# ruppelb/Large-Scale-ViT-SLAM

Hardware: AMD Instinct MI355X
Metric: chunks/sec (16-frame 518x518) + ViT MFMA util% (higher is better)
Workload: dtype bf16; 1 GPU; VGGT aggregator forward (DINOv2-L/14-reg + 24x frame/global AA blocks), 1 chunk of 16 frames 518x518, layers 4/11/17/23 emitted; frames=16, parallelism=replicas x1

## Files before the change

### include/vggt_mi355x.h

```cpp
#ifndef VGGT_MI355X_H
#define VGGT_MI355X_H

#include <stddef.h>
#include <stdint.h>

#ifdef __cplusplus
extern "C" {
#endif

#define VGGT_OK 0
#define VGGT_ERR_SHAPE (-1)
#define VGGT_ERR_ALIGN (-2)
#define VGGT_ERR_HIP (-3)
#define VGGT_ERR_UNSUPPORTED (-4)

#define VGGT_DTYPE_F32 0
#define VGGT_DTYPE_BF16 1

#define VGGT_EPI_BF16 0
#define VGGT_EPI_GELU_BF16 1
#define VGGT_EPI_RESID_F32 2
#define VGGT_EPI_F32 3

#define VGGT_ROPE_NONE 0
#define VGGT_ROPE_2D 1
#define VGGT_ROPE_1D 2

const char* vggt_version(void);

#define VGGT_TUNE_GEMM_TILE 1
#define VGGT_TUNE_ATTN_WAVES 2
#define VGGT_TUNE_ATTN_VARIANT 3
#define VGGT_TUNE_CONV_PF2 4
#define VGGT_TUNE_ATTN16 5
#define VGGT_TUNE_LINEAR_ONE_LAUNCH 6
#define VGGT_TUNE_LINEAR_SPLIT_K 7
#define VGGT_TUNE_LINEAR_WK 8
#define VGGT_TUNE_GEMM_BALANCE 10
#define VGGT_TUNE_ATTN_TAIL_SPLIT 11
int vggt_tune(int knob, int value);

#define VGGT_STREAM_SHORT_WORKGROUPS 1
int vggt_set_stream_config(void* stream, int cus, int flags);

int vggt_gemm_bf16(const void* A, int64_t lda, const void* W, int64_t ldw, const float* bias, int M, int N, int K,
                   int epi, void* out, int64_t ldo, const float* gamma, float* out2, int64_t ldo2, void* stream);

int vggt_gemm_bf16_gelu_pre(const void* A, int64_t lda, const void* W, int64_t ldw, const float* bias, int M, int N,
                            int K, void* out, int64_t ldo, void* pre, int64_t ldp, void* stream);

int vggt_gemm_qkv(const void* A, int64_t lda, const void* W, int64_t ldw, const float* bias, int M, int H, int D, int K,
                  void* out, int64_t ldo, const float* qw, const float* qb, const float* kw, const float* kb, float eps,
                  int rope_mode, const int32_t* pos, int period, const float* cos_tab, const float* sin_tab,
                  int tab_len, void* stream);

int vggt_gemm_headnorm(const void* A, int64_t lda, const void* W, int64_t ldw, const float* bias, int M, int N, int H,
                       int D, int K, void* out, int64_t ldo, const float* nw, const float* nb, float eps, int rope_mode,
                       const int32_t* pos, int period, const float* cos_tab, const float* sin_tab, int tab_len,
                       void* stream);

int vggt_layernorm(const void* x, int in_dtype, int64_t ldx, const float* w, const float* b, float eps, int M, int C,
                   void* y, int out_dtype, int64_t ldy, void* stream);

int vggt_resid_add_layernorm(float* x, int64_t ldx, const void* y, int64_t ldy, const float* gamma, float* out2,
                             int64_t ldo2, const float* w, const float* b, float eps, int M, int C, void* xn,
                             int64_t ldn, void* stream);

int vggt_resid_add_layernorm_nostore(const float* x, int64_t ldx, const void* y, int64_t ldy, const float* gamma,
                                     const float* w, const float* b, float eps, int M, int C, void* xn, int64_t ldn,
                                     void* stream);
int vggt_resid_add2_layernorm(float* x, int64_t ldx, const void* y, int64_t ldy, const float* gamma, const void* y2,
                              int64_t ldy2, const float* gamma2, float* out2, int64_t ldo2, const float* w,
                              const float* b, float eps, int M, int C, void* xn, int64_t ldn, void* stream);

int vggt_headnorm_rope(void* buf, int64_t ld, int col_off, int M, int H, int D, const float* w, const float* b,
                       float eps, int rope_mode, const int32_t* pos, int period, const float* cos_tab,
                       const float* sin_tab, int tab_len, void* stream);

int vggt_qknorm_rope(void* qkv, int64_t ld, int M, int H, int D, const float* qw, const float* qb, const float* kw,
                     const float* kb, float eps, int rope_mode, const int32_t* pos, int period, const float* cos_tab,
                     const float* sin_tab, int tab_len, void* stream);

int vggt_qknorm_rope_out(const void* src, int64_t lds, void* dst, int64_t ldd, int M, int H, int D, const float* qw,
                         const float* qb, const float* kw, const float* kb, float eps, int rope_mode,
                         const int32_t* pos, int period, const float* cos_tab, const float* sin_tab, int tab_len,
                         void* stream);
int vggt_headnorm_rope_out(const void* src, int64_t lds, void* dst, int64_t ldd, int M, int H, int D, const float* w,
                           const float* b, float eps, int rope_mode, const int32_t* pos, int period,
                           const float* cos_tab, const float* sin_tab, int tab_len, void* stream);

int vggt_attention_fwd(const void* q, int64_t ldq, int64_t q_bstride, const void* k, int64_t ldk, int64_t k_bstride,
                       const void* v, int64_t ldv, int64_t v_bstride, void* o, int64_t ldo, int64_t o_bstride,
                       int batch, int heads, int nq, int nk, int D, float scale, void* stream);

int vggt_attention_fwd_ws(const void* q, int64_t ldq, int64_t q_bstride, const void* k, int64_t ldk,
                          int64_t k_bstride, const void* v, int64_t ldv, int64_t v_bstride, void* o, int64_t ldo,
                          int64_t o_bstride, int batch, int heads, int nq, int nk, int D, float scale, void* ws,
                          size_t ws_bytes, void* stream);
size_t vggt_attention_ws_bytes(int batch, int heads, int nq, int nk, int D, void* stream);
int vggt_attention_split_plan(int batch, int heads, int nq, int nk, int D, int cus, int* tail_blocks, int* parts);

int vggt_patch_im2col(const float* images, int F, int H, int W, int patch, const float* mean, const float* std_,
                      void* A, int Kp, void* stream);

int vggt_dino_assemble(const void* patch, const float* cls, const float* reg, const float* pos, int F, int hw,
                       int nreg, int C, float* x, void* stream);

int vggt_special_tokens(float* x, int64_t ldx, int F, int S, int P, int n, int C, const float* tok, void* stream);

int vggt_copy_rows_f32(const float* src, int64_t lds, float* dst, int64_t ldd, int rows, int cols, void* stream);

int vggt_layernorm_grouped(const void* x, int in_dtype, int64_t ldx, const float* w, const float* b, float eps, int M,
                           int C, void* y, int out_dtype, int64_t ldy, int group, int x_group_stride,
                           int x_row_offset, int y_group_stride, int y_row_offset, void* stream);

int vggt_linear_f32(const float* A, int64_t lda, const float* W, int64_t ldw, const float* bias, int M, int N, int K,
                    int act_in, int epi, float* out, int64_t ldo, const float* gamma, void* stream);
int vggt_linear_f32_grouped(const float* A, int64_t lda, int64_t a_gstride, const float* W, int64_t ldw,
                            int64_t w_gstride, const float* bias, int64_t b_gstride, int M, int N, int K, int groups,
                            int act_in, int epi, float* out, int64_t ldo, int64_t o_gstride, void* stream);
int vggt_gated_update_prep(const float* memory, const float* update, int B, int Nt, int D, float* inp, float* g_in,
                           void* stream);
// ... 150 lines not shown
```

### large-scale-vit-slam_amd/aligned_vggt/_native.py

```python
from __future__ import annotations

import ctypes
import os
from typing import Optional

import torch

from .runtime import Workspace, scratch_table

_PKG_ROOT = os.path.dirname(os.path.dirname(os.path.abspath(__file__)))
LIB_PATH = os.environ.get("VGGT_MI355X_LIB", os.path.join(_PKG_ROOT, "lib", "libvggt_mi355x.so"))
HEADER_PATH = os.path.join(os.path.dirname(_PKG_ROOT), "include", "vggt_mi355x.h")

VGGT_OK, VGGT_ERR_SHAPE, VGGT_ERR_ALIGN, VGGT_ERR_HIP, VGGT_ERR_UNSUPPORTED = 0, -1, -2, -3, -4
DTYPE_F32, DTYPE_BF16 = 0, 1
EPI_BF16, EPI_GELU_BF16, EPI_RESID_F32, EPI_F32 = 0, 1, 2, 3
ROPE_NONE, ROPE_2D, ROPE_1D = 0, 1, 2

_ERR = {VGGT_ERR_SHAPE: "unsupported or inconsistent shape", VGGT_ERR_ALIGN: "misaligned pointer or leading dimension",
        VGGT_ERR_HIP: "HIP launch/runtime error", VGGT_ERR_UNSUPPORTED: "unsupported mode or dtype"}

_vp, _i, _i64, _f = ctypes.c_void_p, ctypes.c_int, ctypes.c_int64, ctypes.c_float
_SIGS = {
    "vggt_tune": [_i, _i],
# ... 45 lines not shown
    "vggt_upsample_bilinear_split_sep": [_vp, _i, _i, _i, _i, _vp, _i, _i, _vp, _vp, _vp, _i, _vp],
    "vggt_conv2d_upsample_bf16x3": [_vp, _i, _i, _i, _i, _vp, _i, _i, _vp, _vp, _vp, _i, _i, _vp, _i64, _vp, _vp,
                                    _i64, _i, _vp],
    "vggt_split_act_bf16x2": [_vp, _i64, _i64, _i, _i, _vp, _vp, _vp],
    "vggt_upsample_bilinear_f32": [_vp, _i, _i, _i, _i, _vp, _i, _i, _vp, _vp],
    "vggt_dpt_activate": [_vp, _i64, _i64, _i, _i, _i, _vp, _vp, _vp, _vp],
    "vggt_irls_sim3": [_vp, _i64, _vp, _i64, _vp, _i64, _vp, _i64, _i, _i64, _f, _f, _i, _f, _vp, _vp, _vp, _vp,
                       ctypes.c_size_t, _vp],
    "vggt_sim3_points": [_vp, _i64, _i, _i64, _vp, _vp, _vp, _i64, _vp],
    "vggt_scale_f32": [_vp, _i64, _i, _i64, _vp, _vp],
    "vggt_pose_compose": [_vp, _vp, _vp, _vp, _i, _vp, _i, _i, _i, _i, _i, _vp, _vp, _vp],
    "vggt_attention_fwd_lse": [_vp, _i64, _i64, _vp, _i64, _i64, _vp, _i64, _i64, _vp, _i64, _i64, _vp, _i, _i, _i,
                               _i, _i, _f, _vp],
    "vggt_attention_bwd": [_vp, _i64, _i64, _vp, _i64, _i64, _vp, _i64, _vp, _vp, _i64, _i64, _vp, _vp, _vp, _i64,
                           _vp, _vp, _i64, _i, _i, _i, _i, _i, _f, _vp],
    "vggt_attention_small_bwd": [_vp, _i64, _i64, _vp, _i64, _i64, _vp, _i64, _vp, _i64, _i64, _vp, _i64, _i64, _vp,
                                 _vp, _i64, _i64, _i, _i, _i, _i, _i, _i, _f, _vp],
    "vggt_layernorm_bwd": [_vp, _i, _i64, _vp, _f, _vp, _i, _i64, _vp, _i, _i64, _i, _i, _i, _i, _i, _i, _i, _i, _vp,
                           _vp, _vp, ctypes.c_size_t, _vp],
    "vggt_headnorm_rope_bwd": [_vp, _i64, _vp, _i64, _i, _i, _i, _i, _i, _vp, _vp, _f, _i, _vp, _i, _vp, _vp, _i, _vp,
                               _vp, _vp, _vp, _vp, ctypes.c_size_t, _vp],
    "vggt_colsum": [_vp, _i, _i64, _i, _i, _vp, _i, _vp, ctypes.c_size_t, _vp],
    "vggt_layerscale_bwd": [_vp, _i64, _vp, _i, _i64, _vp, _vp, _i, _i64, _i, _i, _vp, _vp, _vp, ctypes.c_size_t,
                            _vp],
    "vggt_gelu_fwd": [_vp, _i, _i64, _vp, _i, _i64, _i, _i, _vp],
    "vggt_gelu_bwd": [_vp, _i, _i64, _vp, _i, _i64, _vp, _i, _i64, _i, _i, _vp, _vp, ctypes.c_size_t, _vp],
    "vggt_resid_scale_add": [_vp, _i64, _vp, _i, _i64, _vp, _i, _i, _vp],
    "vggt_gemm_bf16_gelu_pre": [_vp, _i64, _vp, _i64, _vp, _i, _i, _i, _vp, _i64, _vp, _i64, _vp],
    "vggt_resid_scale_add_from": [_vp, _i64, _vp, _i64, _vp, _i, _i64, _vp, _i, _i, _vp],
    "vggt_qknorm_rope_out": [_vp, _i64, _vp, _i64, _i, _i, _i, _vp, _vp, _vp, _vp, _f, _i, _vp, _i, _vp, _vp, _i, _vp],
    "vggt_headnorm_rope_out": [_vp, _i64, _vp, _i64, _i, _i, _i, _vp, _vp, _f, _i, _vp, _i, _vp, _vp, _i, _vp],
    "vggt_transpose_b16": [_vp, _i64, _i, _i, _vp, _i64, _i, _vp],
    "vggt_wgrad_f32": [_vp, _i64, _vp, _i64, _i, _i, _i, _vp, _i64, _i, _vp],
    "vggt_wgrad_bias_f32": [_vp, _i64, _vp, _i64, _i, _i, _i, _vp, _i64, _vp, _i, _vp],
    "vggt_wgrad_bf16": [_vp, _i64, _vp, _i64, _i, _i, _i, _vp, _i64, _i, _vp, ctypes.c_size_t, _vp],
    "vggt_batch_dot_f32": [_vp, _vp, _i64, _i, _i64, _vp, _vp, ctypes.c_size_t, _vp],
}
_WS_FNS = {"vggt_colred_workspace_bytes": [_i, _i], "vggt_layernorm_bwd_workspace_bytes": [_i, _i],
           "vggt_headnorm_rope_bwd_workspace_bytes": [_i, _i], "vggt_batch_dot_workspace_bytes": [_i, _i64],
           "vggt_wgrad_bf16_workspace_bytes": [_i, _i, _i], "vggt_attention_ws_bytes": [_i, _i, _i, _i, _i, _vp]}

_lib = None

EVENT_HOOK = None


def lib() -> ctypes.CDLL:
    global _lib
    if _lib is None:
        if not os.path.exists(LIB_PATH):
            raise RuntimeError(f"libvggt_mi355x.so not found at {LIB_PATH}: build it with "
                               f"`make -C large-scale-vit-slam_amd/csrc` (or __graft_entry__.build()); "
                               f"there is no CPU fallback for the HIP hot path")
        L = ctypes.CDLL(LIB_PATH)
        for name, argt in _SIGS.items():
            fn = getattr(L, name)
            fn.argtypes = argt
            fn.restype = ctypes.c_int
        L.vggt_version.restype = ctypes.c_char_p
        L.vggt_irls_workspace_bytes.argtypes = [_i]
        L.vggt_irls_workspace_bytes.restype = ctypes.c_size_t
        for name, argt in _WS_FNS.items():
            fn = getattr(L, name)
            fn.argtypes = argt
            fn.restype = ctypes.c_size_t
        _lib = L
    return _lib


def version() -> str:
    return lib().vggt_version().decode()


TUNE_GEMM_TILE = 1
TUNE_ATTN_WAVES = 2
TUNE_ATTN_VARIANT = 3
TUNE_CONV_PF2 = 4
TUNE_ATTN16 = 5
TUNE_LINEAR_ONE_LAUNCH = 6
TUNE_LINEAR_SPLIT_K = 7
TUNE_LINEAR_WK = 8
TUNE_GEMM_BALANCE = 10
TUNE_ATTN_TAIL_SPLIT = 11


def tune(knob: int, value: int) -> int:
    rc = lib().vggt_tune(knob, value)
    if rc == VGGT_ERR_UNSUPPORTED:
        raise ValueError(f"vggt_tune: unsupported knob/value ({knob}, {value})")
    return rc


STREAM_SHORT_WORKGROUPS = 1


def set_stream_config(stream: int, cus: int, flags: int = 0) -> int:
    rc = lib().vggt_set_stream_config(ctypes.c_void_p(stream), cus, flags)
    if rc < 0:
        raise ValueError(f"vggt_set_stream_config: rejected ({rc})")
    return rc


def mfma_probe(iters: int = 200_000, random: bool = True, seconds: float = 2.0, device=None) -> dict:
    import statistics
    device = torch.device(device or "cuda")
    ncu = torch.cuda.get_device_properties(device).multi_processor_count
    g = torch.Generator(device="cpu").manual_seed(0)
    n = ncu * 256 * 16
    ops = (torch.randn(n, generator=g) if random else torch.zeros(n)).to(torch.bfloat16).to(device)
    stamps = torch.zeros(ncu * 4, dtype=torch.int64, device=device)
    sink = torch.empty(ncu * 256, dtype=torch.float32, device=device)
    st = ctypes.c_void_p(torch.cuda.current_stream(device).cuda_stream)
    launch = lambda: _check(lib().vggt_mfma_probe(_p(stamps), _p(sink), _p(ops), ncu, iters, st),
                            "vggt_mfma_probe")
    import time
    t_end = time.perf_counter() + seconds
    while time.perf_counter() < t_end:
        launch()
        torch.cuda.synchronize(device)
    a = torch.cuda.Event(enable_timing=True)
    b = torch.cuda.Event(enable_timing=True)
    a.record()
    launch()
    b.record()
    b.synchronize()
    ms = a.elapsed_time(b)
    sp = stamps.view(ncu, 4).cpu().tolist()
    clocks = [(t1 - t0) / (r1 - r0) * 100e6 for t0, t1, r0, r1 in sp if r1 > r0]
    clk = statistics.median(clocks)
    flop = ncu * 4 * iters * 8 * 32768.0
    return {"tflops": round(flop / (ms * 1e-3) / 1e12, 1), "clock_ghz": round(clk / 1e9, 3),
            "flop_per_cycle_per_cu": round(flop / ncu / (ms * 1e-3 * clk), 1), "ms": round(ms, 3), "cus": ncu,
            "operands": "random bf16" if random else "zeros"}


def _check(rc: int, name: str) -> None:
    if rc != VGGT_OK:
        raise RuntimeError(f"{name}: {_ERR.get(rc, 'error')} (code {rc})")


def _dev(t: torch.Tensor, name: str) -> None:
    if t.device.type != "cuda":
        raise RuntimeError(f"{name}: tensor on {t.device}; the MI355X hot path runs on HIP devices only")


def _p(t: Optional[torch.Tensor]):
    return None if t is None else ctypes.c_void_p(t.data_ptr())


def _stream() -> ctypes.c_void_p:
    return ctypes.c_void_p(torch.cuda.current_stream().cuda_stream)


def _ld(t: torch.Tensor) -> int:
    if t.dim() != 2 or t.stride(1) != 1:
        raise RuntimeError("expected a 2-D row-major (unit inner stride) view")
    return t.stride(0)


def gemm_bf16(a: torch.Tensor, w: torch.Tensor, bias: torch.Tensor, out: torch.Tensor, epi: int,
              gamma: Optional[torch.Tensor] = None, out2: Optional[torch.Tensor] = None) -> torch.Tensor:
    _dev(a, "gemm_bf16")
    M, K = a.shape
    N = w.shape[0]
    assert a.dtype == torch.bfloat16 and w.dtype == torch.bfloat16 and w.shape[1] == K
    assert out.shape[0] == M and out.shape[1] == N
# ... 705 lines not shown
```

### large-scale-vit-slam_amd/csrc/attention.hip

```cpp
#include <math.h>
#include <stdlib.h>
#include <string.h>

#include <algorithm>
#include <mutex>
#include <type_traits>
#include <vector>

#include "common.h"
#include "tune.h"

namespace {

typedef __attribute__((ext_vector_type(4))) short s16x4;
typedef __attribute__((ext_vector_type(8))) short s16x8;
typedef int int32x4 __attribute__((ext_vector_type(4)));

constexpr int BKV = 64;
constexpr float THR = 8.0f;

struct AttnArgs {
  const bf16_t* q;
  const bf16_t* k;
  const bf16_t* v;
// ... 554 lines not shown
        }
      }
      return nt;
    };
    if constexpr (VAR & 32) {
      const int t1 = run(std::true_type{}, 0);
      if (t1 < nt) run(std::false_type{}, t1);
    } else {
      run(std::false_type{}, 0);
    }
  }

  if constexpr (VAR & 8) {
    l_run = lsum[0];
  } else {
    const auto sw = __builtin_amdgcn_permlane32_swap(__float_as_uint(l_run), __float_as_uint(l_run), false, false);
    l_run = __uint_as_float(sw[0]) + __uint_as_float(sw[1]);
  }
  if constexpr (SPLIT) {
    if (slab >= 0) {
      float* sp = a.ws + (int64_t)slab * SPLIT_SLAB;
#pragma unroll
      for (int db = 0; db < NDB; ++db)
#pragma unroll
        for (int gq = 0; gq < 4; ++gq)
          *(f32x4*)(sp + ((wave * (NDB * 4) + db * 4 + gq) * 64 + lane) * 4) =
              f32x4{o[db][4 * gq], o[db][4 * gq + 1], o[db][4 * gq + 2], o[db][4 * gq + 3]};
      if (hl == 0) *(f32x2*)(sp + BQ * D + (wave * 32 + lane) * 2) = f32x2{m_run, l_run};
      return;
    }
  }
  float inv = 1.f / l_run;
  if constexpr ((VAR & 32) && (VAR & 64)) {
    const auto sw = __builtin_amdgcn_permlane32_swap(__float_as_uint(lb_run), __float_as_uint(lb_run), false, false);
    inv = 1.f / (__uint_as_float(sw[0]) + __uint_as_float(sw[1]));
  }
  if constexpr (VAR & 1024) {
    VGGT_SEG(-1);
    st_acc[6] = st_prev;
    if (lane == 0) {
      unsigned long long* out = (unsigned long long*)(void*)a.lse + ((int64_t)blockIdx.x * NW + wave) * STAMP_N;
#pragma unroll
      for (int i = 0; i < STAMP_N; ++i) out[i] = st_acc[i];
    }
  } else {
    if (a.lse && hl == 0 && qrow < a.nq) a.lse[((int64_t)b * a.heads + h) * a.nq + qrow] = m_run + __log2f(l_run);
  }
  if (qrow < a.nq) {
    bf16_t* op = a.o + ((int64_t)b * a.obs + qrow) * a.ldo + h * D;
#pragma unroll
    for (int db = 0; db < NDB; ++db)
#pragma unroll
      for (int gq = 0; gq < 4; ++gq) {
        uint2 pk;
        pk.x = pack_bf2(o[db][4 * gq] * inv, o[db][4 * gq + 1] * inv);
        pk.y = pack_bf2(o[db][4 * gq + 2] * inv, o[db][4 * gq + 3] * inv);
        *(uint2*)(op + db * 32 + 8 * gq + 4 * hl) = pk;
      }
  }
}

__device__ __forceinline__ int k16_swz(int row, int chunk) { return chunk ^ ((row >> 1) & 7); }
__device__ __forceinline__ int v16_swz(int row, int chunk) { return chunk ^ (((row >> 1) & 3) << 1); }

template <int NW>
__global__ __launch_bounds__(NW * 64, 16 / NW) void attn16_fwd_kernel(AttnArgs a) {
  constexpr int D = 64;
  constexpr int BQ = NW * 32;
  constexpr int ROWB = D * 2;
  constexpr int TILEB = BKV * ROWB;
  constexpr int RPI = 1024 / ROWB;
  constexpr int CPR = ROWB / 16;
  constexpr int IPW = TILEB / 1024 / NW;
  __shared__ __attribute__((aligned(16))) char smem[2 * 2 * TILEB];
  __shared__ int redo;

  const int lane = threadIdx.x & 63;
  const int wave = __builtin_amdgcn_readfirstlane(threadIdx.x >> 6);
  const int g = lane >> 4, c16 = lane & 15;
  if constexpr (NW == 8) {
    if (wave >= 4) __builtin_amdgcn_s_setprio(1);
  }
  const int nqb = (a.nq + BQ - 1) / BQ;
  const int bid = xcd_remap(blockIdx.x, nqb * a.heads * a.batch);
  const int qblk = bid % nqb;
  const int bh = bid / nqb;
  const int h = bh % a.heads;
  const int b = bh / a.heads;

  const bf16_t* qp = a.q + (int64_t)b * a.qbs * a.ldq + h * D;
  const bf16_t* kp = a.k + (int64_t)b * a.kbs * a.ldk + h * D;
  const bf16_t* vp = a.v + (int64_t)b * a.vbs * a.ldv + h * D;
  const int q0 = qblk * BQ + wave * 32 + c16;

  bf16x8 qf[2][2];
#pragma unroll
  for (int qb = 0; qb < 2; ++qb) {
    const int qr = min(q0 + 16 * qb, a.nq - 1);
#pragma unroll
    for (int ks = 0; ks < 2; ++ks) {
      qf[qb][ks] = *(const bf16x8*)(qp + (int64_t)qr * a.ldq + ks * 32 + 8 * g);
#pragma unroll
      for (int j = 0; j < 8; ++j) qf[qb][ks][j] = (__bf16)((float)qf[qb][ks][j] * a.c);
    }
  }
#pragma unroll
  for (int qb = 0; qb < 2; ++qb)
#pragma unroll
    for (int ks = 0; ks < 2; ++ks) asm volatile("" : "+v"(qf[qb][ks]));

  uint32_t koff[IPW], voff[IPW];
#pragma unroll
  for (int i = 0; i < IPW; ++i) {
    const int row = (wave * IPW + i) * RPI + lane / CPR;
    const int cp = lane % CPR;
    koff[i] = (uint32_t)(row * a.ldk + k16_swz(row, cp) * 8) * 2u;
    voff[i] = (uint32_t)(row * a.ldv + v16_swz(row, cp) * 8) * 2u;
  }
  const uint32_t lds0 = __builtin_amdgcn_readfirstlane((uint32_t)(uintptr_t)LDS_PTR(smem)) + wave * IPW * 1024;
  const int kstep = BKV * (int)a.ldk * 2, vstep = BKV * (int)a.ldv * 2;
  const int kbytes = a.nk * (int)a.ldk * 2, vbytes = a.nk * (int)a.ldv * 2;
  auto stage = [&](int buf, int t) {
    const int ko = kstep * t, vo = vstep * t;
    const int32x4 kr = make_rsrc((const char*)kp + ko, (uint32_t)max(kbytes - ko, 0));
    const int32x4 vr = make_rsrc((const char*)vp + vo, (uint32_t)max(vbytes - vo, 0));
    const uint32_t d = lds0 + buf * 2 * TILEB;
#pragma unroll
    for (int i = 0; i < IPW; ++i) {
      dma16(kr, koff[i], d + i * 1024);
      dma16(vr, voff[i], d + TILEB + i * 1024);
    }
  };

  uint32_t ka[2];
#pragma unroll
  for (int ks = 0; ks < 2; ++ks) ka[ks] = c16 * ROWB + (k16_swz(c16, 4 * ks + g) << 4);
  uint32_t va[4];
  {
    const int qq = (lane >> 2) & 3, pp = lane & 3;
    const int r0 = 4 * g + qq;
#pragma unroll
    for (int db = 0; db < 4; ++db) {
      const int col = db * 16 + 4 * pp;
      va[db] = TILEB + r0 * ROWB + (v16_swz(r0, col >> 3) << 4) + (col & 7) * 2;
    }
  }
  const int nt = (a.nk + BKV - 1) / BKV;

  struct S8 {
    f32x4 v[4][2];
  };
  auto scores = [&](auto bufc, int t) -> S8 {
    constexpr int BUF = decltype(bufc)::value;
    const char* base = smem + BUF * 2 * TILEB;
    S8 s;
#pragma unroll
    for (int kb = 0; kb < 4; ++kb) {
      const bf16x8 k0 = *(const bf16x8*)(base + ka[0] + kb * 16 * ROWB);
      const bf16x8 k1 = *(const bf16x8*)(base + ka[1] + kb * 16 * ROWB);
#pragma unroll
      for (int qb = 0; qb < 2; ++qb) {
        s.v[kb][qb] = __builtin_amdgcn_mfma_f32_16x16x32_bf16(k0, qf[qb][0], f32x4{}, 0, 0, 0);
        s.v[kb][qb] = __builtin_amdgcn_mfma_f32_16x16x32_bf16(k1, qf[qb][1], s.v[kb][qb], 0, 0, 0);
      }
    }
    const int kv0 = t * BKV;
    if (kv0 + BKV > a.nk) {
#pragma unroll
      for (int kb = 0; kb < 4; ++kb)
#pragma unroll
        for (int i = 0; i < 4; ++i)
          if (kv0 + kb * 16 + 4 * g + i >= a.nk) {
            s.v[kb][0][i] = -INFINITY;
            s.v[kb][1][i] = -INFINITY;
          }
    }
    return s;
  };

  f32x4 o[4][2];
  float l[2];
  float m[2] = {0.f, 0.f};

  auto soft_pv = [&](auto bufc, int t, auto shc) {
    constexpr int BUF = decltype(bufc)::value;
    constexpr bool SHIFT = decltype(shc)::value;
    const char* base = smem + BUF * 2 * TILEB;
    const S8 s = scores(bufc, t);
    bf16x8 pf[2][2];
#pragma unroll
    for (int qb = 0; qb < 2; ++qb) {
      float rs = 0.f;
#pragma unroll
      for (int kk = 0; kk < 2; ++kk) {
        bf16x8 tv;
#pragma unroll
        for (int j = 0; j < 8; ++j) {
          float x = s.v[2 * kk + (j >> 2)][qb][j & 3];
          if constexpr (SHIFT) x -= m[qb];
          const float p = __builtin_amdgcn_exp2f(x);
          rs += p;
          tv[j] = (__bf16)p;
        }
        pf[qb][kk] = tv;
      }
      l[qb] += rs;
    }
    const char* vb = base;
#pragma unroll
    for (int kk = 0; kk < 2; ++kk)
#pragma unroll
      for (int db = 0; db < 4; ++db) {
        const char* p0 = vb + va[db] + kk * 32 * ROWB;
        const s16x4 lo = __builtin_amdgcn_ds_read_tr16_b64_v4i16((__attribute__((address_space(3))) s16x4*)LDS_PTR(p0));
        const s16x4 hi =
            __builtin_amdgcn_ds_read_tr16_b64_v4i16((__attribute__((address_space(3))) s16x4*)LDS_PTR(p0 + 16 * ROWB));
        const bf16x8 vf = __builtin_bit_cast(bf16x8, (s16x8)__builtin_shufflevector(lo, hi, 0, 1, 2, 3, 4, 5, 6, 7));
#pragma unroll
        for (int qb = 0; qb < 2; ++qb)
          o[db][qb] = __builtin_amdgcn_mfma_f32_16x16x32_bf16(vf, pf[qb][kk], o[db][qb], 0, 0, 0);
      }
  };

  using I0 = std::integral_constant<int, 0>;
  using I1 = std::integral_constant<int, 1>;
  auto sweep = [&](auto body) {
    stage(0, 0);
    asm volatile("s_waitcnt vmcnt(0)" ::: "memory");
    __syncthreads();
    for (int t = 0; t < nt; t += 2) {
      if (t + 1 < nt) stage(1, t + 1);
      body(I0{}, t);
      asm volatile("s_waitcnt vmcnt(0)" ::: "memory");
      __syncthreads();
      if (t + 1 >= nt) break;
      if (t + 2 < nt) stage(0, t + 2);
      body(I1{}, t + 1);
      asm volatile("s_waitcnt vmcnt(0)" ::: "memory");
      __syncthreads();
    }
  };
  auto reset = [&]() {
#pragma unroll
    for (int db = 0; db < 4; ++db)
#pragma unroll
      for (int qb = 0; qb < 2; ++qb) o[db][qb] = f32x4{};
    l[0] = l[1] = 0.f;
  };
  auto allsum = [](float x) {
    const auto s16 = __builtin_amdgcn_permlane16_swap(__float_as_uint(x), __float_as_uint(x), false, false);
    x = __uint_as_float(s16[0]) + __uint_as_float(s16[1]);
    const auto s32 = __builtin_amdgcn_permlane32_swap(__float_as_uint(x), __float_as_uint(x), false, false);
    return __uint_as_float(s32[0]) + __uint_as_float(s32[1]);
  };
  auto allmax = [](float x) {
    const auto s16 = __builtin_amdgcn_permlane16_swap(__float_as_uint(x), __float_as_uint(x), false, false);
    x = fmaxf(__uint_as_float(s16[0]), __uint_as_float(s16[1]));
    const auto s32 = __builtin_amdgcn_permlane32_swap(__float_as_uint(x), __float_as_uint(x), false, false);
    return fmaxf(__uint_as_float(s32[0]), __uint_as_float(s32[1]));
  };

  if (threadIdx.x == 0) redo = 0;
  reset();
  sweep([&](auto bufc, int t) { soft_pv(bufc, t, std::false_type{}); });
  l[0] = allsum(l[0]);
  l[1] = allsum(l[1]);
  const bool bad = !(l[0] >= 0x1p-60f && l[0] <= 0x1p100f) || !(l[1] >= 0x1p-60f && l[1] <= 0x1p100f);
  if (__builtin_amdgcn_ballot_w64(bad) != 0 && lane == 0) redo = 1;
  __syncthreads();
  if (redo) {
    float mx[2] = {-INFINITY, -INFINITY};
    sweep([&](auto bufc, int t) {
      const S8 s = scores(bufc, t);
#pragma unroll
      for (int qb = 0; qb < 2; ++qb)
#pragma unroll
        for (int kb = 0; kb < 4; ++kb)
          mx[qb] = fmaxf(fmaxf(mx[qb], fmaxf(s.v[kb][qb][0], s.v[kb][qb][1])), fmaxf(s.v[kb][qb][2], s.v[kb][qb][3]));
    });
    m[0] = allmax(mx[0]);
    m[1] = allmax(mx[1]);
    reset();
    sweep([&](auto bufc, int t) { soft_pv(bufc, t, std::true_type{}); });
    l[0] = allsum(l[0]);
    l[1] = allsum(l[1]);
  }

#pragma unroll
  for (int qb = 0; qb < 2; ++qb) {
    const int qrow = q0 + 16 * qb;
    const float inv = 1.f / l[qb];
    if (a.lse && g == 0 && qrow < a.nq) a.lse[((int64_t)b * a.heads + h) * a.nq + qrow] = m[qb] + __log2f(l[qb]);
    if (qrow < a.nq) {
      bf16_t* op = a.o + ((int64_t)b * a.obs + qrow) * a.ldo + h * D;
#pragma unroll
      for (int db = 0; db < 4; ++db) {
        uint2 pk;
        pk.x = pack_bf2(o[db][qb][0] * inv, o[db][qb][1] * inv);
        pk.y = pack_bf2(o[db][qb][2] * inv, o[db][qb][3] * inv);
        *(uint2*)(op + db * 16 + 4 * g) = pk;
      }
    }
  }
}

__global__ __launch_bounds__(256) void attn_split_merge_kernel(AttnArgs a, int n_tail) {
  constexpr int D = 64;
  const int tid = blockIdx.x * 256 + threadIdx.x;
  const int lane = tid & 63, c = (tid >> 6) & 7, wave = (tid >> 9) & 7, tu = tid >> 12;
  if (tu >= n_tail) return;
  const int nqb = (a.nq + SPLIT_BQ - 1) / SPLIT_BQ;
  const int bid = a.n_full + tu;
  const int qb = bid % nqb, bh = bid / nqb;
  const int h = bh % a.heads, b = bh / a.heads;
  const int r = wave * 32 + (lane & 31), hl = lane >> 5;
  const int qrow = qb * SPLIT_BQ + r;
  if (qrow >= a.nq) return;
  const float* sp = a.ws + (int64_t)tu * a.parts * SPLIT_SLAB;
  float mx = -INFINITY;
  for (int p = 0; p < a.parts; ++p) mx = fmaxf(mx, sp[(int64_t)p * SPLIT_SLAB + SPLIT_BQ * D + r * 2]);
  f32x4 num = f32x4{0.f, 0.f, 0.f, 0.f};
  float den = 0.f;
  for (int p = 0; p < a.parts; ++p) {
    const float* pp = sp + (int64_t)p * SPLIT_SLAB;
    const f32x2 ml = *(const f32x2*)(pp + SPLIT_BQ * D + r * 2);
    const float w = __builtin_amdgcn_exp2f(ml[0] - mx);
    num += w * *(const f32x4*)(pp + ((wave * 8 + c) * 64 + lane) * 4);
    den += w * ml[1];
  }
  const float inv = 1.f / den;
  uint2 pk;
  pk.x = pack_bf2(num[0] * inv, num[1] * inv);
  pk.y = pack_bf2(num[2] * inv, num[3] * inv);
  bf16_t* op = a.o + ((int64_t)b * a.obs + qrow) * a.ldo + h * D;
  *(uint2*)(op + (c >> 2) * 32 + 8 * (c & 3) + 4 * hl) = pk;
}

inline int attn_cu_count(hipStream_t s) {
  static int dev_cus = [] {
    int dev = 0, n = 0;
    if (hipGetDevice(&dev) != hipSuccess ||
        hipDeviceGetAttribute(&n, hipDeviceAttributeMultiprocessorCount, dev) != hipSuccess || n <= 0)
      n = 256;
    return n;
  }();
  const int n = vggt_stream_cu_count(s);
  return n > 0 ? n : dev_cus;
}

constexpr double PLAN_UNIT_OVH = 2.0;
constexpr double PLAN_TILE_US = 1.87, PLAN_BYTES_PER_US = 3.5e6, PLAN_MERGE_US = 5.0;
constexpr double PLAN_MIN_GAIN = 0.03;
constexpr int PLAN_MIN_PART_TILES = 86;

struct PlanSeg {
  int count;
  double len;
};
double plan_makespan(int cus, const PlanSeg* segs, int nseg) {
  std::vector<double> rem((size_t)cus * 2, 0.0);
  std::vector<int> cnt((size_t)cus, 0);
  int seg = 0, left = nseg > 0 ? segs[0].count : 0, resident = 0;
  double now = 0.0;
  auto more = [&]() {
    while (seg < nseg && left == 0) {
      ++seg;
      if (seg < nseg) left = segs[seg].count;
    }
    return seg < nseg;
  };
  for (;;) {
    for (int want = 0; want < 2; ++want)
      for (int cu = 0; cu < cus; ++cu)
        if (cnt[cu] == want && more()) {
          rem[cu * 2 + cnt[cu]] = segs[seg].len;
          ++cnt[cu];
          --left;
          ++resident;
        }
    if (resident == 0) return now;
    double dt = 1e300;
    for (int cu = 0; cu < cus; ++cu)
      for (int i = 0; i < cnt[cu]; ++i) dt = std::min(dt, rem[cu * 2 + i] * cnt[cu] * 0.5);
    now += dt;
    for (int cu = 0; cu < cus; ++cu) {
      const int n = cnt[cu];
      const double done = dt * 2.0 / (n > 0 ? n : 1);
      int keep = 0;
      for (int i = 0; i < n; ++i) {
        const double r = rem[cu * 2 + i] - done;
        if (r > 1e-9) rem[cu * 2 + keep++] = r;
        else --resident;
      }
      cnt[cu] = keep;
    }
  }
}

inline void split_shape(int nt, int want, int* parts, int* part_tiles) {
  const int p = std::max(1, std::min(want, nt));
  *part_tiles = (nt + p - 1) / p;
  *parts = (nt + *part_tiles - 1) / *part_tiles;
}

}

extern "C" int vggt_attention_split_plan(int batch, int heads, int nq, int nk, int D, int cus, int* tail_blocks,
                                         int* parts) {
  if (tail_blocks) *tail_blocks = 0;
  if (parts) *parts = 0;
  if (batch <= 0 || heads <= 0 || nq < 4096 || nk <= 0 || D != 64 || cus <= 0) return 0;
  const int64_t units64 = (int64_t)((nq + SPLIT_BQ - 1) / SPLIT_BQ) * heads * batch;
  const int slots = 2 * cus, nt = (nk + BKV - 1) / BKV;
  if (units64 < slots || units64 > (1 << 24) || units64 % slots == 0 || nt < 2) return 0;
  const int units = (int)units64, tail = units % slots;
  struct Entry {
    int key[4], tail, parts;
  };
  static std::mutex mu;
  static std::vector<Entry> cache;
  const int key[4] = {units, nq, nk, cus};
  std::lock_guard<std::mutex> lk(mu);
  const Entry* hit = nullptr;
  for (const Entry& e : cache)
    if (!memcmp(e.key, key, sizeof key)) hit = &e;
  if (!hit) {
    const PlanSeg whole[1] = {{units, nt + PLAN_UNIT_OVH}};
    const double t0 = plan_makespan(cus, whole, 1);
    double best = t0;
    int best_p = 0;
    for (int want = 2; want <= 4; ++want) {
      int p, pt;
// ... 13 lines not shown
  if (hit->parts < 2) return 0;
  if (tail_blocks) *tail_blocks = hit->tail;
  if (parts) *parts = hit->parts;
  return 1;
}

namespace {
void tail_split_of(int batch, int heads, int nq, int nk, int cus, int* tail, int* parts, int* part_tiles) {
  *tail = *parts = *part_tiles = 0;
  const int knob = g_vggt_attn_tail_split;
  const int64_t units = (int64_t)((nq + SPLIT_BQ - 1) / SPLIT_BQ) * heads * batch;
  const int nt = (nk + BKV - 1) / BKV;
  int t = 0, p = 0;
  if (knob < 0 || units > (1 << 18)) return;
  if (knob > 0) {
    p = knob & 0xff;
    t = (int)std::min<int64_t>(knob >> 8, units);
  } else if (!vggt_attention_split_plan(batch, heads, nq, nk, 64, cus, &t, &p)) {
    return;
  }
  int pr, pt;
  split_shape(nt, std::min(p, 4), &pr, &pt);
  if (pr < 2 || t <= 0) return;
  *tail = t;
  *parts = pr;
  *part_tiles = pt;
}

bool attn_split_path(int nq, int D) {
  static const bool dma_half = getenv("VGGT_ATTN_DMA_HALF") ? atoi(getenv("VGGT_ATTN_DMA_HALF")) != 0 : true;
  return dma_half && g_vggt_attn_variant == 33 && D == 64 && g_vggt_attn_waves == 8 && nq >= 4096;
}
}

extern "C" size_t vggt_attention_ws_bytes(int batch, int heads, int nq, int nk, int D, void* stream) {
  if (batch <= 0 || heads <= 0 || nq <= 0 || nk <= 0 || !attn_split_path(nq, D)) return 0;
  int tail, parts, pt;
  tail_split_of(batch, heads, nq, nk, attn_cu_count((hipStream_t)stream), &tail, &parts, &pt);
  return (size_t)tail * parts * SPLIT_SLAB * sizeof(float);
}

static int attention_fwd_impl(const void* q, int64_t ldq, int64_t q_bstride, const void* k, int64_t ldk,
                              int64_t k_bstride, const void* v, int64_t ldv, int64_t v_bstride, void* o, int64_t ldo,
                              int64_t o_bstride, int batch, int heads, int nq, int nk, int D, float scale, void* ws,
                              size_t ws_bytes, void* stream);

extern "C" int vggt_attention_fwd(const void* q, int64_t ldq, int64_t q_bstride, const void* k, int64_t ldk,
                                  int64_t k_bstride, const void* v, int64_t ldv, int64_t v_bstride, void* o,
                                  int64_t ldo, int64_t o_bstride, int batch, int heads, int nq, int nk, int D,
                                  float scale, void* stream) {
  return attention_fwd_impl(q, ldq, q_bstride, k, ldk, k_bstride, v, ldv, v_bstride, o, ldo, o_bstride, batch, heads,
                            nq, nk, D, scale, nullptr, 0, stream);
}

extern "C" int vggt_attention_fwd_ws(const void* q, int64_t ldq, int64_t q_bstride, const void* k, int64_t ldk,
                                     int64_t k_bstride, const void* v, int64_t ldv, int64_t v_bstride, void* o,
                                     int64_t ldo, int64_t o_bstride, int batch, int heads, int nq, int nk, int D,
                                     float scale, void* ws, size_t ws_bytes, void* stream) {
  if (ws && (uintptr_t)ws % 16) return VGGT_ERR_ALIGN;
  return attention_fwd_impl(q, ldq, q_bstride, k, ldk, k_bstride, v, ldv, v_bstride, o, ldo, o_bstride, batch, heads,
                            nq, nk, D, scale, ws, ws_bytes, stream);
}

static int attention_fwd_impl(const void* q, int64_t ldq, int64_t q_bstride, const void* k, int64_t ldk,
                              int64_t k_bstride, const void* v, int64_t ldv, int64_t v_bstride, void* o, int64_t ldo,
                              int64_t o_bstride, int batch, int heads, int nq, int nk, int D, float scale, void* ws,
                              size_t ws_bytes, void* stream) {
  if (batch <= 0 || heads <= 0 || nq <= 0 || nk <= 0) return VGGT_ERR_SHAPE;
  if (D != 64 && D != 128) return VGGT_ERR_UNSUPPORTED;
  if ((ldq | ldk | ldv | ldo) % 8 || ((uintptr_t)q | (uintptr_t)k | (uintptr_t)v | (uintptr_t)o) % 16)
    return VGGT_ERR_ALIGN;
  if ((uint64_t)nk * (uint64_t)(ldk > ldv ? ldk : ldv) * 2 >= (1ull << 31)) return VGGT_ERR_SHAPE;
  AttnArgs a{(const bf16_t*)q, (const bf16_t*)k, (const bf16_t*)v, (bf16_t*)o, ldq, ldk, ldv, ldo,
             q_bstride, k_bstride, v_bstride, o_bstride, batch, heads, nq, nk,
             scale * 1.4426950408889634f, nullptr};
  const bool two_ok = (g_vggt_attn_variant & 32) && (g_vggt_attn_variant & 65) == 1;
  const int nw = (g_vggt_attn_waves == 8 && nq >= 4096) ? 8 : (g_vggt_attn_waves == 2 && two_ok) ? 2 : 4;
  const int nwg = ((nq + nw * 32 - 1) / (nw * 32)) * heads * batch;
  hipStream_t s = (hipStream_t)stream;
  const bool use16 = a.lse == nullptr && D == 64 && nw != 2 &&
                     (g_vggt_attn_variant == 161 ||
                      (g_vggt_attn_variant == 33 && (g_vggt_attn16 == 1 || (g_vggt_attn16 == 2 && nw == 4))));
  if (use16) {
    if (nw == 8) attn16_fwd_kernel<8><<<nwg, 512, 0, s>>>(a);
    else attn16_fwd_kernel<4><<<nwg, 256, 0, s>>>(a);
    HIP_LAUNCH_CHECK();
    return VGGT_OK;
  }
  if ((g_vggt_attn_variant == 19 || g_vggt_attn_variant == 23) && D == 64 && nw != 2) {
    if (nw == 8 && g_vggt_attn_variant == 23) attn_fwd_kernel<64, 8, 23><<<nwg, 512, 0, s>>>(a);
    else if (nw == 8) attn_fwd_kernel<64, 8, 19><<<nwg, 512, 0, s>>>(a);
    else if (g_vggt_attn_variant == 23) attn_fwd_kernel<64, 4, 23><<<nwg, 256, 0, s>>>(a);
    else attn_fwd_kernel<64, 4, 19><<<nwg, 256, 0, s>>>(a);
    HIP_LAUNCH_CHECK();
    return VGGT_OK;
  }
  static const bool dma_half = getenv("VGGT_ATTN_DMA_HALF") ? atoi(getenv("VGGT_ATTN_DMA_HALF")) != 0 : true;
  if (dma_half && g_vggt_attn_variant == 33 && D == 64 && nw == 8 && !a.lse) {
    int tail = 0, parts = 0, pt = 0;
    if (ws) tail_split_of(batch, heads, nq, nk, attn_cu_count(s), &tail, &parts, &pt);
    if (parts >= 2) {
      if (ws_bytes < (size_t)tail * parts * SPLIT_SLAB * sizeof(float)) return VGGT_ERR_SHAPE;
      a.n_full = nwg - tail;
      a.parts = parts;
      a.part_tiles = pt;
      a.ws = (float*)ws;
      attn_fwd_kernel<64, 8, 2081 | 8192><<<a.n_full + tail * parts, 512, 0, s>>>(a);
      HIP_LAUNCH_CHECK();
      attn_split_merge_kernel<<<tail * 16, 256, 0, s>>>(a, tail);
      HIP_LAUNCH_CHECK();
      return VGGT_OK;
    }
    attn_fwd_kernel<64, 8, 2081><<<nwg, 512, 0, s>>>(a);
    HIP_LAUNCH_CHECK();
    return VGGT_OK;
  }
  if (g_vggt_attn_variant == 4129 && D == 64 && nw != 2 && !a.lse) {
    if (nw == 8) attn_fwd_kernel<64, 8, 4129><<<nwg, 512, 0, s>>>(a);
    else attn_fwd_kernel<64, 4, 33><<<nwg, 256, 0, s>>>(a);
    HIP_LAUNCH_CHECK();
    return VGGT_OK;
  }
  if (g_vggt_attn_variant == 2081 && D == 64 && nw != 2 && !a.lse) {
    if (nw == 8) attn_fwd_kernel<64, 8, 2081><<<nwg, 512, 0, s>>>(a);
    else attn_fwd_kernel<64, 4, 33><<<nwg, 256, 0, s>>>(a);
    HIP_LAUNCH_CHECK();
    return VGGT_OK;
  }
  if (g_vggt_attn_variant == 545 && D == 64 && nw != 2 && !a.lse) {
    if (nw == 8) attn_fwd_kernel<64, 8, 545><<<nwg, 512, 0, s>>>(a);
    else attn_fwd_kernel<64, 4, 545><<<nwg, 256, 0, s>>>(a);
    HIP_LAUNCH_CHECK();
    return VGGT_OK;
  }
  if (g_vggt_attn_variant == 289 && D == 64 && nw != 2 && !a.lse) {
    if (nw == 8) attn_fwd_kernel<64, 8, 289><<<nwg, 512, 0, s>>>(a);
    else attn_fwd_kernel<64, 4, 289><<<nwg, 256, 0, s>>>(a);
    HIP_LAUNCH_CHECK();
    return VGGT_OK;
  }
  if (g_vggt_attn_variant & 32) {
    const int v = (g_vggt_attn_variant & 1) + ((g_vggt_attn_variant & 64) ? 2 : 0);
    switch ((D == 64 ? 0 : 16) + (nw == 8 ? 4 : nw == 2 ? 8 : 0) + v) {
#define VGGT_ATTN_SCASE(DD, NWW, V)                                                               \
  case (DD == 64 ? 0 : 16) + (NWW == 8 ? 4 : NWW == 2 ? 8 : 0) + V:                                \
    attn_fwd_kernel<DD, NWW, 32 + (V & 1) + ((V & 2) ? 64 : 0)><<<nwg, NWW * 64, 0, s>>>(a); \
    break;
      VGGT_ATTN_SCASE(64, 4, 0) VGGT_ATTN_SCASE(64, 4, 1) VGGT_ATTN_SCASE(64, 4, 2) VGGT_ATTN_SCASE(64, 4, 3)
      VGGT_ATTN_SCASE(64, 8, 0) VGGT_ATTN_SCASE(64, 8, 1) VGGT_ATTN_SCASE(64, 8, 2) VGGT_ATTN_SCASE(64, 8, 3)
      VGGT_ATTN_SCASE(128, 4, 0) VGGT_ATTN_SCASE(128, 4, 1) VGGT_ATTN_SCASE(128, 4, 2) VGGT_ATTN_SCASE(128, 4, 3)
      VGGT_ATTN_SCASE(128, 8, 0) VGGT_ATTN_SCASE(128, 8, 1) VGGT_ATTN_SCASE(128, 8, 2) VGGT_ATTN_SCASE(128, 8, 3)
      VGGT_ATTN_SCASE(64, 2, 1) VGGT_ATTN_SCASE(128, 2, 1)
#undef VGGT_ATTN_SCASE
      default: return VGGT_ERR_UNSUPPORTED;
    }
    HIP_LAUNCH_CHECK();
    return VGGT_OK;
  }
  switch ((D == 64 ? 0 : 32) + (nw == 8 ? 16 : 0) + (g_vggt_attn_variant & 15)) {
#define VGGT_ATTN_CASE(DD, NWW, V) \
  case (DD == 64 ? 0 : 32) + (NWW == 8 ? 16 : 0) + V: attn_fwd_kernel<DD, NWW, V><<<nwg, NWW * 64, 0, s>>>(a); break;
#define VGGT_ATTN_CASES(DD, NWW)                                                                            \
  VGGT_ATTN_CASE(DD, NWW, 0) VGGT_ATTN_CASE(DD, NWW, 1) VGGT_ATTN_CASE(DD, NWW, 2) VGGT_ATTN_CASE(DD, NWW, 3)  \
  VGGT_ATTN_CASE(DD, NWW, 4) VGGT_ATTN_CASE(DD, NWW, 5) VGGT_ATTN_CASE(DD, NWW, 6) VGGT_ATTN_CASE(DD, NWW, 7)  \
  VGGT_ATTN_CASE(DD, NWW, 8) VGGT_ATTN_CASE(DD, NWW, 9) VGGT_ATTN_CASE(DD, NWW, 10) VGGT_ATTN_CASE(DD, NWW, 11) \
  VGGT_ATTN_CASE(DD, NWW, 12) VGGT_ATTN_CASE(DD, NWW, 13) VGGT_ATTN_CASE(DD, NWW, 14) VGGT_ATTN_CASE(DD, NWW, 15)
    VGGT_ATTN_CASES(64, 4)
    VGGT_ATTN_CASES(64, 8)
// ... 54 lines not shown
```

### large-scale-vit-slam_amd/csrc/capi.cpp

```cpp
#include "../../include/vggt_mi355x.h"

extern "C" const char* vggt_version(void) { return "vggt_mi355x 0.1 gfx950"; }

#include <stdlib.h>

#include <atomic>
#include <mutex>

#include "tune.h"

namespace {
int env_or(const char* name, int dflt) {
  const char* e = getenv(name);
  return e ? atoi(e) : dflt;
}
}

int g_vggt_gemm_tile = env_or("VGGT_GEMM", -1);
int g_vggt_attn_waves = env_or("VGGT_ATTN_WAVES", 8);
int g_vggt_attn_variant = env_or("VGGT_ATTN_VARIANT", 33);
int g_vggt_attn16 = env_or("VGGT_ATTN16", 2);
int g_vggt_conv_pf2 = env_or("VGGT_CONV_PF2", 1);
int g_vggt_linear_one_launch = env_or("VGGT_LINEAR_ONE_LAUNCH", 1);
int g_vggt_linear_split_k = env_or("VGGT_LINEAR_SPLIT_K", 128);
int g_vggt_linear_wk = env_or("VGGT_LINEAR_WK", 64);
int g_vggt_gemm_balance = env_or("VGGT_GEMM_BALANCE", 0);
int g_vggt_attn_tail_split = env_or("VGGT_ATTN_TAIL_SPLIT", -1);

extern "C" int vggt_tune(int knob, int value) {
  int prev;
  switch (knob) {
    case VGGT_TUNE_GEMM_TILE:
      if (value < -1 || value > 9) return VGGT_ERR_UNSUPPORTED;
      prev = g_vggt_gemm_tile;
      g_vggt_gemm_tile = value;
      return prev;
    case VGGT_TUNE_ATTN_WAVES:
      if (value != 2 && value != 4 && value != 8) return VGGT_ERR_UNSUPPORTED;
      prev = g_vggt_attn_waves;
      g_vggt_attn_waves = value;
      return prev;
    case VGGT_TUNE_ATTN_VARIANT:
      if (value < 0 || (value > 15 && value != 19 && value != 23 && value != 32 && value != 33 && value != 96 &&
                        value != 97 && value != 161 && value != 289 && value != 545 && value != 2081 && value != 4129))
        return VGGT_ERR_UNSUPPORTED;
      prev = g_vggt_attn_variant;
      g_vggt_attn_variant = value;
      return prev;
    case VGGT_TUNE_ATTN16:
      if (value < 0 || value > 2) return VGGT_ERR_UNSUPPORTED;
      prev = g_vggt_attn16;
      g_vggt_attn16 = value;
      return prev;
    case VGGT_TUNE_LINEAR_ONE_LAUNCH:
      if (value != 0 && value != 1) return VGGT_ERR_UNSUPPORTED;
      prev = g_vggt_linear_one_launch;
      g_vggt_linear_one_launch = value;
      return prev;
    case VGGT_TUNE_LINEAR_SPLIT_K:
      if (value < 16 || value > 4096 || (value & (value - 1))) return VGGT_ERR_UNSUPPORTED;
      prev = g_vggt_linear_split_k;
      g_vggt_linear_split_k = value;
      return prev;
    case VGGT_TUNE_LINEAR_WK:
      if (value != 0 && (value < 64 || value > 4096 || (value & (value - 1)))) return VGGT_ERR_UNSUPPORTED;
      prev = g_vggt_linear_wk;
      g_vggt_linear_wk = value;
      return prev;
    case VGGT_TUNE_GEMM_BALANCE:
      if (value != 0 && value != 1) return VGGT_ERR_UNSUPPORTED;
      prev = g_vggt_gemm_balance;
      g_vggt_gemm_balance = value;
      return prev;
    case VGGT_TUNE_ATTN_TAIL_SPLIT:
      if (value < -1 || (value > 0 && ((value & 0xff) < 2 || (value >> 8) < 1))) return VGGT_ERR_UNSUPPORTED;
      prev = g_vggt_attn_tail_split;
      g_vggt_attn_tail_split = value;
      return prev;
    case VGGT_TUNE_CONV_PF2:
      if (value != 0 && value != 1) return VGGT_ERR_UNSUPPORTED;
      prev = g_vggt_conv_pf2;
      g_vggt_conv_pf2 = value;
      return prev;
    default: return VGGT_ERR_UNSUPPORTED;
  }
}

namespace {
constexpr int kMaxStreams = 16;
std::atomic<void*> g_cfg_stream[kMaxStreams];
std::atomic<int> g_cfg_cus[kMaxStreams];
std::atomic<int> g_cfg_flags[kMaxStreams];
std::mutex g_cfg_mu;
int find_cfg(void* stream) {
  if (!stream) return -1;
  for (int i = 0; i < kMaxStreams; ++i)
    if (g_cfg_stream[i].load(std::memory_order_acquire) == stream) return i;
  return -1;
}
}

int vggt_stream_cu_count(void* stream) {
  const int i = find_cfg(stream);
  return i < 0 ? 0 : g_cfg_cus[i].load(std::memory_order_relaxed);
}

int vggt_stream_flags(void* stream) {
  const int i = find_cfg(stream);
  return i < 0 ? 0 : g_cfg_flags[i].load(std::memory_order_relaxed);
}

extern "C" int vggt_set_stream_config(void* stream, int cus, int flags) {
  if (!stream || cus < 0 || (flags & ~VGGT_STREAM_SHORT_WORKGROUPS)) return VGGT_ERR_SHAPE;
  std::lock_guard<std::mutex> lk(g_cfg_mu);
  int slot = find_cfg(stream);
  const int prev = slot < 0 ? 0 : (g_cfg_cus[slot].load(std::memory_order_relaxed) |
                                    g_cfg_flags[slot].load(std::memory_order_relaxed) << 16);
  if (cus == 0 && flags == 0) {
    if (slot >= 0) g_cfg_stream[slot].store(nullptr, std::memory_order_release);
    return prev;
  }
  if (slot < 0) {
    for (int i = 0; i < kMaxStreams && slot < 0; ++i)
      if (!g_cfg_stream[i].load(std::memory_order_relaxed)) slot = i;
    if (slot < 0) return VGGT_ERR_UNSUPPORTED;
    g_cfg_cus[slot].store(cus, std::memory_order_relaxed);
    g_cfg_flags[slot].store(flags, std::memory_order_relaxed);
    g_cfg_stream[slot].store(stream, std::memory_order_release);
  } else {
    g_cfg_cus[slot].store(cus, std::memory_order_relaxed);
    g_cfg_flags[slot].store(flags, std::memory_order_relaxed);
  }
  return prev;
}
```

### large-scale-vit-slam_amd/csrc/tune.h

```cpp
#pragma once
extern int g_vggt_gemm_tile;
extern int g_vggt_attn_waves;
extern int g_vggt_attn_variant;
extern int g_vggt_attn16;
extern int g_vggt_conv_pf2;
extern int g_vggt_linear_split_k;
extern int g_vggt_linear_one_launch;
extern int g_vggt_linear_wk;
extern int g_vggt_gemm_balance;
extern int g_vggt_attn_tail_split;
int vggt_stream_cu_count(void* stream);
int vggt_stream_flags(void* stream);
```

Baseline: 10.82 chunks/s.

## Add persistent-grid mode to attn16 kernel and vectorize output stores

Turns the attn16 forward kernel into a grid-stride loop over (q-block, head, batch) items so it can run as a persistent grid sized from CU count times occupancy, behind a new tune knob that defaults to off. The redo flag now uses a per-item stamp so it stays correct across iterations. Output stores are rewritten to use permlane16_swap and 128-bit buffer stores with bounds clamping, replacing per-lane 64-bit stores, and this path runs by default. A shape guard rejects oversized output strides.

```diff
diff --git a/include/vggt_mi355x.h b/include/vggt_mi355x.h
--- a/include/vggt_mi355x.h
+++ b/include/vggt_mi355x.h
@@ -38,6 +38,7 @@
 #define VGGT_TUNE_LINEAR_WK 8
 #define VGGT_TUNE_GEMM_BALANCE 10
 #define VGGT_TUNE_ATTN_TAIL_SPLIT 11
+#define VGGT_TUNE_ATTN16_PERSIST 12
 int vggt_tune(int knob, int value);
 
 #define VGGT_STREAM_SHORT_WORKGROUPS 1
diff --git a/large-scale-vit-slam_amd/aligned_vggt/_native.py b/large-scale-vit-slam_amd/aligned_vggt/_native.py
--- a/large-scale-vit-slam_amd/aligned_vggt/_native.py
+++ b/large-scale-vit-slam_amd/aligned_vggt/_native.py
@@ -151,6 +151,7 @@
 TUNE_LINEAR_WK = 8
 TUNE_GEMM_BALANCE = 10
 TUNE_ATTN_TAIL_SPLIT = 11
+TUNE_ATTN16_PERSIST = 12
 
 
 def tune(knob: int, value: int) -> int:
diff --git a/large-scale-vit-slam_amd/csrc/attention.hip b/large-scale-vit-slam_amd/csrc/attention.hip
--- a/large-scale-vit-slam_amd/csrc/attention.hip
+++ b/large-scale-vit-slam_amd/csrc/attention.hip
@@ -660,32 +660,36 @@
     if (wave >= 4) __builtin_amdgcn_s_setprio(1);
   }
   const int nqb = (a.nq + BQ - 1) / BQ;
-  const int bid = xcd_remap(blockIdx.x, nqb * a.heads * a.batch);
-  const int qblk = bid % nqb;
-  const int bh = bid / nqb;
-  const int h = bh % a.heads;
-  const int b = bh / a.heads;
-
-  const bf16_t* qp = a.q + (int64_t)b * a.qbs * a.ldq + h * D;
-  const bf16_t* kp = a.k + (int64_t)b * a.kbs * a.ldk + h * D;
-  const bf16_t* vp = a.v + (int64_t)b * a.vbs * a.ldv + h * D;
-  const int q0 = qblk * BQ + wave * 32 + c16;
-
+  const int items = nqb * a.heads * a.batch;
+
+  int qblk, h, b;
+  const bf16_t *kp, *vp;
   bf16x8 qf[2][2];
-#pragma unroll
-  for (int qb = 0; qb < 2; ++qb) {
-    const int qr = min(q0 + 16 * qb, a.nq - 1);
-#pragma unroll
-    for (int ks = 0; ks < 2; ++ks) {
-      qf[qb][ks] = *(const bf16x8*)(qp + (int64_t)qr * a.ldq + ks * 32 + 8 * g);
-#pragma unroll
-      for (int j = 0; j < 8; ++j) qf[qb][ks][j] = (__bf16)((float)qf[qb][ks][j] * a.c);
-    }
-  }
-#pragma unroll
-  for (int qb = 0; qb < 2; ++qb)
-#pragma unroll
-    for (int ks = 0; ks < 2; ++ks) asm volatile("" : "+v"(qf[qb][ks]));
+  auto begin_item = [&](int it) {
+    const int bid = xcd_remap(it, items);
+    qblk = bid % nqb;
+    const int bh = bid / nqb;
+    h = bh % a.heads;
+    b = bh / a.heads;
+    const bf16_t* qp = a.q + (int64_t)b * a.qbs * a.ldq + h * D;
+    kp = a.k + (int64_t)b * a.kbs * a.ldk + h * D;
+    vp = a.v + (int64_t)b * a.vbs * a.ldv + h * D;
+    const int q0 = qblk * BQ + wave * 32 + c16;
+#pragma unroll
+    for (int qb = 0; qb < 2; ++qb) {
+      const int qr = min(q0 + 16 * qb, a.nq - 1);
+#pragma unroll
+      for (int ks = 0; ks < 2; ++ks) {
+        qf[qb][ks] = *(const bf16x8*)(qp + (int64_t)qr * a.ldq + ks * 32 + 8 * g);
+#pragma unroll
+        for (int j = 0; j < 8; ++j) qf[qb][ks][j] = (__bf16)((float)qf[qb][ks][j] * a.c);
+      }
+    }
+#pragma unroll
+    for (int qb = 0; qb < 2; ++qb)
+#pragma unroll
+      for (int ks = 0; ks < 2; ++ks) asm volatile("" : "+v"(qf[qb][ks]));
+  };
 
   uint32_t koff[IPW], voff[IPW];
 #pragma unroll
@@ -782,6 +786,7 @@
         }
         pf[qb][kk] = tv;
       }
+      asm("" : "+v"(rs));
       l[qb] += rs;
     }
     const char* vb = base;
@@ -838,45 +843,56 @@
     return fmaxf(__uint_as_float(s32[0]), __uint_as_float(s32[1]));
   };
 
+  typedef __attribute__((ext_vector_type(4))) unsigned int u32x4;
   if (threadIdx.x == 0) redo = 0;
-  reset();
-  sweep([&](auto bufc, int t) { soft_pv(bufc, t, std::false_type{}); });
-  l[0] = allsum(l[0]);
-  l[1] = allsum(l[1]);
-  const bool bad = !(l[0] >= 0x1p-60f && l[0] <= 0x1p100f) || !(l[1] >= 0x1p-60f && l[1] <= 0x1p100f);
-  if (__builtin_amdgcn_ballot_w64(bad) != 0 && lane == 0) redo = 1;
-  __syncthreads();
-  if (redo) {
-    float mx[2] = {-INFINITY, -INFINITY};
-    sweep([&](auto bufc, int t) {
-      const S8 s = scores(bufc, t);
-#pragma unroll
-      for (int qb = 0; qb < 2; ++qb)
-#pragma unroll
-        for (int kb = 0; kb < 4; ++kb)
-          mx[qb] = fmaxf(fmaxf(mx[qb], fmaxf(s.v[kb][qb][0], s.v[kb][qb][1])), fmaxf(s.v[kb][qb][2], s.v[kb][qb][3]));
-    });
-    m[0] = allmax(mx[0]);
-    m[1] = allmax(mx[1]);
+  for (int it = blockIdx.x, stamp = 1; it < items; it += (int)gridDim.x, ++stamp) {
+    begin_item(it);
+    m[0] = m[1] = 0.f;
     reset();
-    sweep([&](auto bufc, int t) { soft_pv(bufc, t, std::true_type{}); });
+    sweep([&](auto bufc, int t) { soft_pv(bufc, t, std::false_type{}); });
     l[0] = allsum(l[0]);
     l[1] = allsum(l[1]);
-  }
-
-#pragma unroll
-  for (int qb = 0; qb < 2; ++qb) {
-    const int qrow = q0 + 16 * qb;
-    const float inv = 1.f / l[qb];
-    if (a.lse && g == 0 && qrow < a.nq) a.lse[((int64_t)b * a.heads + h) * a.nq + qrow] = m[qb] + __log2f(l[qb]);
-    if (qrow < a.nq) {
-      bf16_t* op = a.o + ((int64_t)b * a.obs + qrow) * a.ldo + h * D;
-#pragma unroll
-      for (int db = 0; db < 4; ++db) {
-        uint2 pk;
-        pk.x = pack_bf2(o[db][qb][0] * inv, o[db][qb][1] * inv);
-        pk.y = pack_bf2(o[db][qb][2] * inv, o[db][qb][3] * inv);
-        *(uint2*)(op + db * 16 + 4 * g) = pk;
+    const bool bad = !(l[0] >= 0x1p-60f && l[0] <= 0x1p100f) || !(l[1] >= 0x1p-60f && l[1] <= 0x1p100f);
+    if (__builtin_amdgcn_ballot_w64(bad) != 0 && lane == 0) redo = stamp;
+    __syncthreads();
+    if (redo == stamp) {
+      float mx[2] = {-INFINITY, -INFINITY};
+      sweep([&](auto bufc, int t) {
+        const S8 s = scores(bufc, t);
+#pragma unroll
+        for (int qb = 0; qb < 2; ++qb)
+#pragma unroll
+          for (int kb = 0; kb < 4; ++kb)
+            mx[qb] = fmaxf(fmaxf(mx[qb], fmaxf(s.v[kb][qb][0], s.v[kb][qb][1])), fmaxf(s.v[kb][qb][2], s.v[kb][qb][3]));
+      });
+      m[0] = allmax(mx[0]);
+      m[1] = allmax(mx[1]);
+      reset();
+      sweep([&](auto bufc, int t) { soft_pv(bufc, t, std::true_type{}); });
+      l[0] = allsum(l[0]);
+      l[1] = allsum(l[1]);
+    }
+
+    const int rows = min(a.nq - qblk * BQ, BQ);
+    const __amdgpu_buffer_rsrc_t ro = __builtin_amdgcn_make_buffer_rsrc(
+        (void*)(a.o + ((int64_t)b * a.obs + qblk * BQ) * a.ldo + h * D), 0, ((rows - 1) * (int)a.ldo + D) * 2,
+        0x00020000);
+#pragma unroll
+    for (int qb = 0; qb < 2; ++qb) {
+      const int rl = wave * 32 + c16 + 16 * qb;
+      const float inv = 1.f / l[qb];
+      if (a.lse && g == 0 && rl < rows)
+        a.lse[((int64_t)b * a.heads + h) * a.nq + qblk * BQ + rl] = m[qb] + __log2f(l[qb]);
+#pragma unroll
+      for (int db = 0; db < 4; db += 2) {
+        const uint32_t a0 = pack_bf2(o[db][qb][0] * inv, o[db][qb][1] * inv);
+        const uint32_t a1 = pack_bf2(o[db][qb][2] * inv, o[db][qb][3] * inv);
+        const uint32_t b0 = pack_bf2(o[db + 1][qb][0] * inv, o[db + 1][qb][1] * inv);
+        const uint32_t b1 = pack_bf2(o[db + 1][qb][2] * inv, o[db + 1][qb][3] * inv);
+        const auto s0 = __builtin_amdgcn_permlane16_swap(a0, b0, false, false);
+        const auto s1 = __builtin_amdgcn_permlane16_swap(a1, b1, false, false);
+        const u32x4 pk = {s0[0], s1[0], s0[1], s1[1]};
+        __builtin_amdgcn_raw_buffer_store_b128(pk, ro, (rl * (int)a.ldo + (db + (g & 1)) * 16 + (g >> 1) * 8) * 2, 0, 0);
       }
     }
   }
@@ -926,6 +942,20 @@
   return n > 0 ? n : dev_cus;
 }
 
+inline int attn16_resident(int nw) {
+  static const int r4 = [] {
+    int n = 0;
+    return hipOccupancyMaxActiveBlocksPerMultiprocessor(&n, attn16_fwd_kernel<4>, 256, 0) == hipSuccess && n > 0
+               ? n : 4;
+  }();
+  static const int r8 = [] {
+    int n = 0;
+    return hipOccupancyMaxActiveBlocksPerMultiprocessor(&n, attn16_fwd_kernel<8>, 512, 0) == hipSuccess && n > 0
+               ? n : 2;
+  }();
+  return nw == 8 ? r8 : r4;
+}
+
 constexpr double PLAN_UNIT_OVH = 2.0;
 constexpr double PLAN_TILE_US = 1.87, PLAN_BYTES_PER_US = 3.5e6, PLAN_MERGE_US = 5.0;
 constexpr double PLAN_MIN_GAIN = 0.03;
@@ -1105,8 +1135,14 @@
                      (g_vggt_attn_variant == 161 ||
                       (g_vggt_attn_variant == 33 && (g_vggt_attn16 == 1 || (g_vggt_attn16 == 2 && nw == 4))));
   if (use16) {
-    if (nw == 8) attn16_fwd_kernel<8><<<nwg, 512, 0, s>>>(a);
-    else attn16_fwd_kernel<4><<<nwg, 256, 0, s>>>(a);
+    if (ldo * (nw * 32) * 2 >= (1ll << 31)) return VGGT_ERR_SHAPE;
+    int grid = nwg;
+    if (g_vggt_attn16_persist != 0 && !(vggt_stream_flags(s) & VGGT_STREAM_SHORT_WORKGROUPS)) {
+      grid = std::min(nwg, attn_cu_count(s) * attn16_resident(nw));
+      if (g_vggt_attn16_persist >= 2) grid = std::min(grid, g_vggt_attn16_persist);
+    }
+    if (nw == 8) attn16_fwd_kernel<8><<<grid, 512, 0, s>>>(a);
+    else attn16_fwd_kernel<4><<<grid, 256, 0, s>>>(a);
     HIP_LAUNCH_CHECK();
     return VGGT_OK;
   }
diff --git a/large-scale-vit-slam_amd/csrc/capi.cpp b/large-scale-vit-slam_amd/csrc/capi.cpp
--- a/large-scale-vit-slam_amd/csrc/capi.cpp
+++ b/large-scale-vit-slam_amd/csrc/capi.cpp
@@ -26,6 +26,7 @@
 int g_vggt_linear_wk = env_or("VGGT_LINEAR_WK", 64);
 int g_vggt_gemm_balance = env_or("VGGT_GEMM_BALANCE", 0);
 int g_vggt_attn_tail_split = env_or("VGGT_ATTN_TAIL_SPLIT", -1);
+int g_vggt_attn16_persist = env_or("VGGT_ATTN16_PERSIST", 0);
 
 extern "C" int vggt_tune(int knob, int value) {
   int prev;
@@ -76,6 +77,11 @@
       if (value < -1 || (value > 0 && ((value & 0xff) < 2 || (value >> 8) < 1))) return VGGT_ERR_UNSUPPORTED;
       prev = g_vggt_attn_tail_split;
       g_vggt_attn_tail_split = value;
+      return prev;
+    case VGGT_TUNE_ATTN16_PERSIST:
+      if (value < 0) return VGGT_ERR_UNSUPPORTED;
+      prev = g_vggt_attn16_persist;
+      g_vggt_attn16_persist = value;
       return prev;
     case VGGT_TUNE_CONV_PF2:
       if (value != 0 && value != 1) return VGGT_ERR_UNSUPPORTED;
diff --git a/large-scale-vit-slam_amd/csrc/tune.h b/large-scale-vit-slam_amd/csrc/tune.h
--- a/large-scale-vit-slam_amd/csrc/tune.h
+++ b/large-scale-vit-slam_amd/csrc/tune.h
@@ -9,5 +9,6 @@
 extern int g_vggt_linear_wk;
 extern int g_vggt_gemm_balance;
 extern int g_vggt_attn_tail_split;
+extern int g_vggt_attn16_persist;
 int vggt_stream_cu_count(void* stream);
 int vggt_stream_flags(void* stream);
```

New measurement: 10.86 chunks/s, median of 3. About the same (+0.4%).
